# SimonRennotte/Data-Efficient-Reinforcement-Learning-with-Probabilistic-Model-Predictive-Control

Measured on AMD Instinct MI355X. Metric: MPC trajectory rollouts/sec, higher is better.
Workload: dtype f64

## Files before the change

### data-efficient-reinforcement-learning-with-probabilistic-model-predictive-control_amd/_lib.py

```python
import ctypes as C
import os

_HERE = os.path.dirname(os.path.abspath(__file__))
LIB_PATH = os.environ.get("GPMPC_LIB") or os.path.join(_HERE, "libgpmpc_hip.so")

GPMPC_OK = 0
GPMPC_ERR_ARG = -1
GPMPC_ERR_NOT_PD = -2
GPMPC_ERR_HIP = -3
GPMPC_ERR_LIMIT = -4


class GpmpcError(RuntimeError):
    def __init__(self, code, msg):
        super().__init__(f"gpmpc error {code}: {msg}")
        self.code = code


class NotPositiveDefiniteError(GpmpcError):
    """Cholesky failure of K + noise*I -- the reference lets torch.linalg.cholesky's error
    propagate uncaught (rl_gp_mpc/control_objects/models/gp_model.py:427)."""


_P = C.c_void_p
# ... 49 lines not shown
    "gpmpc_lbfgs_state_size": (C.c_longlong, [_I, _I, _I]),
    "gpmpc_lbfgs_init": (C.c_int, [_P, _P, _I, _I, _I, _I, _I, _P, _P, _P, _P]),
    "gpmpc_lbfgs_step": (C.c_int, [_P, _P, _P, _I, _I, _I, _I, _I, _D, _D, _I, _P, _P, _P, _P]),
    "gpmpc_lbfgs_search": (C.c_int, [_P, _P, _P, _I, _I, _I, _I, _D, _I, _I, _I, _I, _D, _D, _I, _P, _P, _P, _P, _P, _P]),
    "gpmpc_mll_batch": (C.c_int, [_P, _P, _P, _I, _I, _I, _P, _I, _P, _P, _I, _P, _P, _P, _P, _P]),
    "gpmpc_train_search": (C.c_int, [_P, _P, _P, _I, _I, _I, _I, _P, _P, _I, _I, _I, _I, _D, _D, _P, _P, _P, _P]),
    "gpmpc_ilqr_state_size": (C.c_longlong, [_I, _I, _I, _I, _I]),
    "gpmpc_ilqr_backward": (C.c_int, [_P, _P, _P, _I, _I, _I, _I, _D, _P, _P, _P, _P, _P, _P]),
    "gpmpc_ilqr_forward": (C.c_int, [_P, _P, _P, _P, _P, _P, _I, _I, _I, _I, _D, _P, _I, _P, _P, _P, _P]),
    "gpmpc_ilqr_init": (C.c_int, [_P, _P, _I, _I, _I, _I, _D, _P, _P]),
    "gpmpc_ilqr_step": (C.c_int, [_P, _P, _I, _I, _I, _I, _D, _I, _D, _D, _D, _D, _P, _P]),
    "gpmpc_ilqr_search": (C.c_int, [_P, _P, _P, _I, _I, _I, _I, _D, _I, _I, _D, _D, _D, _D, _P, _P, _P, _P]),
    "gpmpc_argmin_async": (C.c_int, [_P, _P, _I, C.c_longlong, _P, _I, _P, _P]),
    "gpmpc_argmin_export": (C.c_int, [_P, _P, _I, C.c_longlong, _P, _I, _P, _P, _P]),
    "gpmpc_argmin": (C.c_int, [_P, _P, _I, C.c_longlong, C.POINTER(_D), C.POINTER(C.c_longlong), _P]),
}


ABI_VERSION = 29


def load(path=LIB_PATH):
    if not os.path.exists(path):
        raise ImportError(
            f"{path} not found: the HIP extension is required (no CPU fallback). "
            "Build it with `python __graft_entry__.py` or `make -C <package>/csrc`.")
    lib = C.CDLL(path)
    for name, (res, args) in SIGNATURES.items():
        fn = getattr(lib, name)
        fn.restype = res
        fn.argtypes = args
    if lib.gpmpc_abi_version() != ABI_VERSION:
        raise ImportError(f"{path}: ABI version {lib.gpmpc_abi_version()} != expected {ABI_VERSION}; rebuild the HIP library")
    return lib
# ... 11 lines not shown
```

### data-efficient-reinforcement-learning-with-probabilistic-model-predictive-control_amd/csrc/abi.hip

```cpp
#include <climits>
#include <cmath>
#include <cstring>
#include <new>
#include <dlfcn.h>

#include "gpmpc_internal.h"
#include "lqr_gains_plan.h"
#include "lbfgs_state.h"
#include "ilqr_state.h"

namespace {
struct Roctx {
    int (*push)(const char*) = nullptr;
    int (*pop)() = nullptr;
    Roctx() {
        for (const char* lib : {"librocprofiler-sdk-roctx.so", "libroctx64.so"}) {
            void* hnd = dlopen(lib, RTLD_LAZY | RTLD_LOCAL);
            if (!hnd) continue;
            push = reinterpret_cast<int (*)(const char*)>(dlsym(hnd, "roctxRangePushA"));
            pop = reinterpret_cast<int (*)()>(dlsym(hnd, "roctxRangePop"));
            if (push && pop) return;
            push = nullptr; pop = nullptr;
        }
    }
// ... 105 lines not shown
}

template <class Run>
static int query_entry(gpmpc_t* g, const char* name, const char* count_name, int count, int D, int E, bool check_limits,
                       bool have_ptrs, Run run) {
    int rc = query_checks(g, name, count_name, count, D, E, check_limits);
    if (rc) return rc;
    if (count > 0 && !have_ptrs) return bad(g, "null argument");
    if (count == 0) return GPMPC_OK;
    GPMPC_HIP_CHECK(H_(g), hipSetDevice(g->h.device));
    return run(H_(g));
}

extern "C" {

int gpmpc_abi_version(void) { return 29; }

int gpmpc_create(gpmpc_t** out, int device_id) {
    if (!out) return GPMPC_ERR_ARG;
    *out = nullptr;
    int ndev = 0;
    if (hipGetDeviceCount(&ndev) != hipSuccess || device_id < 0 || device_id >= ndev) return GPMPC_ERR_HIP;
    if (hipSetDevice(device_id) != hipSuccess) return GPMPC_ERR_HIP;
    gpmpc_t* g = new (std::nothrow) gpmpc();
    if (!g) return GPMPC_ERR_HIP;
    g->h.device = device_id;
    hipDeviceProp_t prop;
    if (hipGetDeviceProperties(&prop, device_id) == hipSuccess) {
        g->h.num_cu = prop.multiProcessorCount;
        if (prop.maxSharedMemoryPerMultiProcessor >= 64 * 1024)
            g->h.lds_limit = (int)prop.maxSharedMemoryPerMultiProcessor;
// ... 1 lines not shown
    }
    *out = g;
    return GPMPC_OK;
}

int gpmpc_destroy(gpmpc_t* g) {
    if (!g) return GPMPC_ERR_ARG;
    Handle* h = H_(g);
    (void)hipSetDevice(h->device);
    Buf* all[] = {&h->Xt, &h->beta, &h->iK, &h->Tm, &h->ils2, &h->var, &h->logvar, &h->gram,
                  &h->linv, &h->zvec, &h->cost, &h->best, &h->xrange, &h->mono_w, &h->traj, &h->Xc, &h->Yc,
                  &h->hyp, &h->kv, &h->vv, &h->sc, &h->gradws, &h->mllws, &h->mllbws, &h->trainws, &h->cemws, &h->tilews, &h->sepw, &h->tgradws, &h->xch, &h->hio, &h->predws, &h->predbws, &h->covws, &h->momws, &h->mombws, &h->linws, &h->linbws, &h->fbws, &h->fbbws, &h->lqrws, &h->lbfgsws, &h->ilqrws, &h->Xf, &h->Yf, &h->fgws, &h->spws, &h->sprec, &h->selws, &h->spupd};
    for (Buf* b : all) free_buf(*b);
    if (h->hio_host) (void)hipHostFree(h->hio_host);
    if (h->hio_flag) (void)hipHostFree(h->hio_flag);
    if (h->xch_uc) (void)hipFree(h->xch_uc);
    if (h->info) (void)hipFree(h->info);
    if (h->fidx) (void)hipFree(h->fidx);
    if (h->mono_exp) (void)hipFree(h->mono_exp);
    if (h->septab) (void)hipFree(h->septab);
    if (h->side_stream) (void)hipStreamDestroy(h->side_stream);
    if (h->ev_params) (void)hipEventDestroy(h->ev_params);
    if (h->ev_points) (void)hipEventDestroy(h->ev_points);
    delete g;
    return GPMPC_OK;
}

const char* gpmpc_last_error(const gpmpc_t* g) { return g ? g->h.err.c_str() : "null handle"; }

int gpmpc_set_option(gpmpc_t* g, const char* name, long long value) {
// ... 220 lines not shown
    memcpy(a.mu0, mu0, h->D * sizeof(double));
    memcpy(a.S0, S0, (size_t)h->D * h->D * sizeof(double));
    return GPMPC_OK;
}

static int rollout_entry(gpmpc_t* g, bool linear, const double* actions, const double* gains, int gains_per_candidate,
                         const double* mu0, const double* S0, int B, int H, int A, int include_time, double time0, double* mu_out,
                         double* Sig_out, double* cm_out, double* cv_out, double* J_out, void* stream) {
    if (!g) return GPMPC_ERR_ARG;
    RolloutArgs a;
    int rc = fill_args(g, a, actions, mu0, S0, B, H, A, include_time, time0, cm_out || cv_out || J_out);
    if (rc) return rc;
    if (gains && A < 1) return bad(g, "feedback gains need A >= 1");
    GPMPC_HIP_CHECK(H_(g), hipSetDevice(g->h.device));
    a.mu_out = mu_out; a.Sig_out = Sig_out; a.cm_out = cm_out; a.cv_out = cv_out; a.J_out = J_out;
    if (!linear) return launch_rollout(H_(g), a, (hipStream_t)stream);
    return run_rollout_linear(H_(g), a, (hipStream_t)stream, gains, gains && gains_per_candidate != 0);
}

int gpmpc_rollout(gpmpc_t* g, const double* actions, const double* mu0, const double* S0, int B, int H, int A,
                  int include_time, double time0, double* mu_out, double* Sig_out, double* cm_out, double* cv_out,
                  double* J_out, void* stream) {
    Range roctx_range("gpmpc_rollout");
    return rollout_entry(g, false, actions, nullptr, 0, mu0, S0, B, H, A, include_time, time0, mu_out, Sig_out, cm_out, cv_out, J_out,
                         stream);
}

int gpmpc_rollout_linear(gpmpc_t* g, const double* actions, const double* mu0, const double* S0, int B, int H, int A,
                         int include_time, double time0, double* mu_out, double* Sig_out, double* cm_out, double* cv_out,
                         double* J_out, void* stream) {
// ... 120 lines not shown
    if (!actions_bar_out) return bad(g, "null argument");
    if (!gains && gains_bar_out) return bad(g, "gains_bar_out without gains");
    RolloutSeeds sd{mu_bar, Sig_bar, cm_bar, cv_bar, J_bar, mu0_bar_out, S0_bar_out, cm_bar || cv_bar || J_bar};
    RolloutArgs a;
    int rc = fill_args(g, a, actions, mu0, S0, B, H, A, include_time, time0, sd.cost);
    if (rc) return rc;
    if (A < 1) return bad(g, "gradient needs A >= 1");
    if (a.D > GPMPC_MAX_D || a.E > GPMPC_MAX_E) {
        g->h.err = "rollout_feedback_backward: D or E beyond the compiled limits";
        return GPMPC_ERR_LIMIT;
    }
    GPMPC_HIP_CHECK(H_(g), hipSetDevice(g->h.device));
    return run_rollout_feedback_backward(H_(g), a, sd, gains, gains && gains_per_candidate != 0, actions_bar_out, gains_bar_out,
                                         (hipStream_t)stream);
}

namespace {
constexpr int kUploadMax = 480;
struct UploadArgs { double v[kUploadMax]; };
__global__ __launch_bounds__(64) void upload_kernel(double* dst, int n, const UploadArgs a) {
    for (int i = threadIdx.x; i < n; i += 64) dst[i] = a.v[i];
}
}

int gpmpc_objective_grad_host(gpmpc_t* g, const double* actions_host, const double* mu0, const double* S0, int H, int A,
                              int include_time, double time0, const double** result_host, void* stream) {
    Range roctx_range("gpmpc_objective_grad_host");
    if (!g) return GPMPC_ERR_ARG;
    if (!actions_host || !result_host) return bad(g, "null argument");
    Handle* h = H_(g);
// ... 42 lines not shown
    a.Sig_out = q; q += (size_t)(H + 1) * D * D;
    a.cm_out = q; q += H + 1;
    a.cv_out = q;
    const unsigned long long seq = ++h->hio_seq;
    const bool sweep_exports = D <= 8;
    h->hx_out = h->hio_host_dev; h->hx_src = out_dev; h->hx_n = sweep_exports ? (int)n_out : 0;
    rc = launch_rollout_grad(h, a, grad, s);
    h->hx_n = 0;
    if (rc) return rc;
    if (!sweep_exports) {
        GPMPC_HIP_CHECK(h, hipStreamSynchronize(s));
        GPMPC_HIP_CHECK(h, hipMemcpy(h->hio_host, out_dev, n_out * sizeof(double), hipMemcpyDeviceToHost));
        *result_host = h->hio_host;
        return GPMPC_OK;
    }
    volatile unsigned long long* flag = h->hio_flag;
    for (unsigned spins = 1; *flag != seq; ++spins) {
        __builtin_ia32_pause();
        if ((spins & 0xfff) == 0) {
            const hipError_t qe = hipStreamQuery(s);
            if (qe == hipSuccess) {
                if (*flag == seq) break;
                h->err = "objective_grad_host: the launches ended without the sweep's completion word";
                return GPMPC_ERR_HIP;
            }
            if (qe != hipErrorNotReady) GPMPC_HIP_CHECK(h, qe);
        }
    }
    __atomic_thread_fence(__ATOMIC_ACQUIRE);
    *result_host = h->hio_host;
    return GPMPC_OK;
}

int gpmpc_cem_search(gpmpc_t* g, const double* mu0, const double* S0, int B, int H, int A, int include_time, double time0,
                     int iterations, int n_elite, unsigned long long seed, const double* first_candidate, int mapper,
                     const double* max_change, const double* action_prev, const double* noise_dev, double* best_out_dev,
                     void* stream) {
    Range roctx_range("gpmpc_cem_search");
    if (!g) return GPMPC_ERR_ARG;
    if (!best_out_dev) return bad(g, "null argument");
    Handle* h = H_(g);
    if (!h->ready) return bad(g, "search before prepare / set_factors");
    RolloutArgs a;
    int rc = fill_args(g, a, best_out_dev, mu0, S0, B, H, A, include_time, time0);
// ... 285 lines not shown
                        double* out_host, void* stream) {
    Range roctx_range("gpmpc_argmin_export");
    if (!g || !J || !out_dev || !out_host || B < 1 || first < 0 || HA < 0) return bad(g, "bad argument");
    Handle* h = H_(g);
    GPMPC_HIP_CHECK(h, hipSetDevice(h->device));
    hipPointerAttribute_t attr;
    void* dev_view = nullptr;
    if (hipPointerGetAttributes(&attr, out_host) != hipSuccess || attr.type != hipMemoryTypeHost ||
        hipHostGetDevicePointer(&dev_view, out_host, 0) != hipSuccess || !dev_view) {
        (void)hipGetLastError();
        return bad(g, "out_host must be pinned (page-locked, device-mapped) host memory");
    }
    return launch_argmin_to(h, J, B, first, actions, HA, out_dev, static_cast<double*>(dev_view), (hipStream_t)stream);
}

static int sparse_update_entry(gpmpc_t* g, const char* name, const double* X, const double* Y, int k, int D, int E, bool forget,
                               void* stream) {
    if (!g) return GPMPC_ERR_ARG;
    Handle* h = H_(g);
    const std::string pre = std::string(name) + ": ";
    if (!h->ready || !h->sp_have) return bad(g, (pre + "the handle holds no record of a gpmpc_prepare_sparse").c_str());
    if (!X || !Y) return bad(g, "null argument");
    if (k < 1) return bad(g, (pre + "need k >= 1 points").c_str());
    if (D != h->D || E != h->E) return bad(g, (pre + "D and E must be those of the cached sparse model").c_str());
    GPMPC_HIP_CHECK(h, hipSetDevice(h->device));
    return run_sparse_update(h, X, Y, k, forget, (hipStream_t)stream);
}

int gpmpc_sparse_append(gpmpc_t* g, const double* Xnew, const double* Ynew, int k, int D, int E, void* stream) {
    Range roctx_range("gpmpc_sparse_append");
// ... 10 lines not shown
```

### data-efficient-reinforcement-learning-with-probabilistic-model-predictive-control_amd/csrc/gpmpc_internal.h

```cpp
#pragma once
#include <hip/hip_runtime.h>
#include <cstddef>
#include <cstdio>
#include <string>
#include <unordered_set>

#include "../../include/gpmpc.h"

namespace gpmpc_hip {

constexpr int kMaxD = GPMPC_MAX_D;
constexpr int kMaxE = GPMPC_MAX_E;
constexpr int kWave = 64;

struct ClusterMap {
    int CS, D, P, P_off, wpp, wtri, koff;
    int CSd;
    unsigned char sepown[8];
    unsigned char meanown[4];
    unsigned char dmem[32];
    unsigned char didx[32];
    __host__ __device__ int diag_owner(int ord, int slot) const { return dmem[((ord * wtri + slot) * CSd) / (D * wtri)]; }
    __host__ __device__ int off_owner(int ord, int slot) const { return ((slot * koff) / wpp + ord * koff) % CS; }
    __host__ __device__ int sep_owner(int ord) const { return sepown[ord]; }
// ... 94 lines not shown
    int t_begin, t_end;
    int ntiles;
    const double* tile_part;
    const int* slow;
    double* grad_mom;
    int* grad_done;
    int grad_NSP, grad_NXP;
    int cluster;
    ClusterMap cmap;
    int cl_slots;
    int xch_n;
    unsigned xch_tag0;
    unsigned long long* xch;
    unsigned long long* xch_uc;
    int cl_dbg;
    int act_inline_n;
    double* act_store;
    double act_inline[kInlineActs];
    double mu0[kMaxD];
    double S0[kMaxD * kMaxD];
};

inline void rollout_objective_only(RolloutArgs& a, const double* actions, double* J) {
    a.actions = actions;
    a.J_out = J;
    a.mu_out = nullptr; a.Sig_out = nullptr; a.cm_out = nullptr; a.cv_out = nullptr;
}

struct Buf {
    double* p = nullptr;
// ... 52 lines not shown
    bool have_state = false;
    Buf Xf, Yf;
    Buf fgws;
    Buf spws;
    Buf selws;
    int* fidx = nullptr;
    size_t fidx_cap = 0;
    Buf hio;
    double* hio_host = nullptr;
    double* hio_host_dev = nullptr;
    size_t hio_host_cap = 0;
    unsigned long long* hio_flag = nullptr;
    unsigned long long* hio_flag_dev = nullptr;
    unsigned long long hio_seq = 0;
    double* hx_out = nullptr; const double* hx_src = nullptr; int hx_n = 0;
    Buf xch;
    unsigned long long* xch_uc = nullptr;
    size_t xch_uc_cap = 0;
    unsigned xch_epoch = 1;
    int opt_cluster = 0;
    int opt_cl_dbg = 0;
    int last_cluster = 1;
    int last_pair_groups = 1;
    Buf mono_w;
    int* mono_exp = nullptr;
    int mono_D = -1;
    int mono_cum[16] = {0};
    int sep_kmax = 0;
    int mono_CM = 0;
    int* info = nullptr;
// ... 155 lines not shown
    SyrkInvForm syrk;
};

struct ForgetRows {
    int k;
    int few[8];
    const int* many;
};

int ensure_rollout_tables(Handle* h, int N, int D);
int plan_rollout(const Handle& h, int N, int D, int A, int E, int H, int Bp, const RolloutRequest& req, RolloutPlan& p);
int launch_rollout(Handle* h, RolloutArgs& a, const RolloutPlan& p, hipStream_t s);
int launch_rollout(Handle* h, RolloutArgs& a, hipStream_t s);
int launch_argmin(Handle* h, const double* J, int B, long long first, hipStream_t s);
int launch_traj_cost(Handle* h, const RolloutArgs& a, double* cm, double* cv, double* J, hipStream_t s);
int ensure_sep_table(Handle* h, int D);
bool tile_path_fits(const Handle& h, int N, int D, int E);
int tile_workspace(Handle* h, RolloutArgs& a);
int launch_tile_state_init(Handle* h, const RolloutArgs& a, hipStream_t s);
int launch_pair_tiles(Handle* h, const RolloutArgs& a, int t, hipStream_t s);
bool tile_moments_supported(const Handle& h, int D, int E, int NSP);
int launch_tile_moments(Handle* h, const RolloutArgs& a, double* mom, int* done, int NSP, int NXP, hipStream_t s);
struct RolloutSeeds {
    const double* mu; const double* Sig; const double* cm; const double* cv; const double* J;
    double* mu0_bar; double* S0_bar;
    bool cost;
};
int plan_rollout_grad(Handle* h, int N, int D, int A, int E, int H, int B, int Bp, bool seeded, GradPlan& p);
int launch_rollout_grad(Handle* h, RolloutArgs& a, double* grad_out, hipStream_t s, const RolloutSeeds* seeds = nullptr);
int launch_rollout_grad_wide(Handle* h, RolloutArgs& a, double* grad_out, hipStream_t s,
// ... 95 lines not shown
```

### data-efficient-reinforcement-learning-with-probabilistic-model-predictive-control_amd/csrc/moments_linear.hip

```cpp
#include "moments_linear_kernels.h"

namespace gpmpc_hip {

namespace {

struct LinFinishArgs {
    const double* part;
    const double* ils2;
    const double* var;
    const double* Sig;
    double* M_out;
    double* S_out;
    double* V_out;
    int rows, E, D, nCB, NW;
    long long Mc;
};

__global__ __launch_bounds__(64) void moments_linear_finish_kernel(LinFinishArgs p) {
    __shared__ double s_sum[kMaxD][kMaxE + 2];
    __shared__ double s_V[kMaxE][kMaxD];
    __shared__ double s_T[kMaxE][kMaxD];
    const int m = blockIdx.x, tid = threadIdx.x;
    const int D = p.D, E = p.E, NW = p.NW;
    const bool with_S = p.S_out != nullptr;
// ... 115 lines not shown
        }
        double ucb = -cm + kappa * sqrt(cv);
        if (clip) ucb = fmin(ucb, 0.0);
        jsum -= ucb;
        if (cm_out) cm_out[(size_t)c * (H + 1) + t] = cm;
        if (cv_out) cv_out[(size_t)c * (H + 1) + t] = cv;
    }
    jsum = wave_xor_sum(jsum);
    if (lane == 0 && J_out) J_out[c] = jsum / (double)(H + 1);
}

}

int launch_traj_cost_feedback(Handle* h, const RolloutArgs& a, int rows, const double* mu, const double* Sig, const double* actions,
                              const double* gains, long long gain_stride, double* cm, double* cv, double* J, hipStream_t s) {
    const int D = a.D, A = a.A, H = a.H;
    auto launch = [&](auto kernel) {
        hipLaunchKernelGGL(kernel, dim3(rows), dim3(64), 0, s, mu, Sig, actions, gains, gain_stride, a.cost, D, A, H, a.kappa,
                           a.clip, a.use_constraints, cm, cv, J);
    };
    static_assert(kMaxD <= 16, "traj_cost_feedback_kernel: per-lane arrays");
    if (D <= 4) launch(traj_cost_feedback_kernel<4>);
    else if (D <= 8) launch(traj_cost_feedback_kernel<8>);
    else launch(traj_cost_feedback_kernel<16>);
    GPMPC_HIP_CHECK(h, hipGetLastError());
    return GPMPC_OK;
}

int run_moments_linear(Handle* h, const double* mu, const double* Sig, int P, double* M_out, double* S_out, double* V_out,
                       hipStream_t s) {
// ... 89 lines not shown
```

### data-efficient-reinforcement-learning-with-probabilistic-model-predictive-control_amd/csrc/rollout.hip

```cpp
#include "rollout_stream_kernel.h"

namespace gpmpc_hip {

int launch_rollout_dp2(Handle*, RolloutArgs&, int, bool, size_t, hipStream_t);
int launch_rollout_dp3(Handle*, RolloutArgs&, int, bool, size_t, hipStream_t);
int launch_rollout_dp4(Handle*, RolloutArgs&, int, bool, size_t, hipStream_t);
int launch_rollout_dp6(Handle*, RolloutArgs&, int, bool, size_t, hipStream_t);
int launch_rollout_dp8(Handle*, RolloutArgs&, int, bool, size_t, hipStream_t);
int launch_rollout_dp16(Handle*, RolloutArgs&, int, bool, size_t, hipStream_t);

__global__ __launch_bounds__(64) void traj_cost_kernel(const double* __restrict__ mu, const double* __restrict__ Sig,
                                                       const double* __restrict__ actions, const double* __restrict__ cost,
                                                       int D, int A, int H, double kappa, int clip, int use_constraints,
                                                       double* __restrict__ cm_out, double* __restrict__ cv_out,
                                                       double* __restrict__ J_out) {
    traj_cost_body(blockIdx.x, threadIdx.x, mu, Sig, actions, cost, D, A, H, kappa, clip, use_constraints, cm_out, cv_out, J_out);
}

__device__ __forceinline__ void keep_better(double& bv, long long& bi, double ov, long long oi) {
    if (oi >= 0 && (bi < 0 || ov < bv || (ov == bv && oi < bi))) { bv = ov; bi = oi; }
}

__global__ __launch_bounds__(1024) void argmin_kernel(const double* J, int B, long long first, double* out, int index_as_double,
                                                     const double* actions, int HA, double* out_host) {
// ... 33 lines not shown
        if (index_as_double) out[1] = (double)gi;
        else reinterpret_cast<long long*>(out)[1] = gi;
        if (out_host) { out_host[0] = bv; out_host[1] = (double)gi; }
    }
    if (actions) {
        const long long w = bi < 0 ? 0 : bi;
        for (int k = tid; k < HA; k += nt) {
            const double v = actions[w * HA + k];
            out[2 + k] = v;
            if (out_host) out_host[2 + k] = v;
        }
    }
    if (out_host) __threadfence_system();
}

__global__ __launch_bounds__(256) void xch_zero_kernel(unsigned long long* p, size_t n) {
    for (size_t i = (size_t)blockIdx.x * 256 + threadIdx.x; i < n; i += (size_t)gridDim.x * 256)
        __hip_atomic_store(p + i, 0ull, __ATOMIC_RELAXED, __HIP_MEMORY_SCOPE_AGENT);
}

struct InlineActs { double v[kInlineActs]; };
__global__ __launch_bounds__(64) void inline_acts_kernel(double* dst, int n, const InlineActs a) {
    for (int i = threadIdx.x; i < n; i += 64) dst[i] = a.v[i];
}

static int zero_exchange(Handle* h, unsigned long long* p, size_t words, hipStream_t s) {
    const unsigned blocks = (unsigned)((words + 255) / 256 < 256 ? (words + 255) / 256 : 256);
    hipLaunchKernelGGL(xch_zero_kernel, dim3(blocks ? blocks : 1), dim3(256), 0, s, p, words);
    GPMPC_HIP_CHECK(h, hipGetLastError());
    return GPMPC_OK;
}

int launch_traj_cost(Handle* h, const RolloutArgs& a, double* cm, double* cv, double* J, hipStream_t s) {
    hipLaunchKernelGGL(traj_cost_kernel, dim3(a.B), dim3(64), 0, s, a.mu_out, a.Sig_out, a.actions, a.cost, a.D, a.A, a.H, a.kappa,
                       a.clip, a.use_constraints, cm, cv, J);
    GPMPC_HIP_CHECK(h, hipGetLastError());
    return GPMPC_OK;
}

static inline int argmin_threads(int B) {
    const int w = (B + 63) / 64;
    return 64 * (w < 1 ? 1 : w > 16 ? 16 : w);
}

int launch_argmin_to(Handle* h, const double* J, int B, long long first, const double* actions, int HA, double* out_dev,
                     double* out_host, hipStream_t s) {
    hipLaunchKernelGGL(argmin_kernel, dim3(1), dim3(argmin_threads(B)), 0, s, J, B, first, out_dev, 1, actions, HA, out_host);
    GPMPC_HIP_CHECK(h, hipGetLastError());
    return GPMPC_OK;
}

// ... 280 lines not shown
        }
    };
    if (tiled) {
        rc = tile_workspace(h, a);
        if (!rc) rc = launch_tile_state_init(h, a, s);
        for (int t = 0; t < a.H && !rc; ++t) {
            rc = launch_pair_tiles(h, a, t, s);
            a.t_begin = t; a.t_end = t + 1;
            if (!rc) rc = launch_kernel();
        }
    } else {
        rc = launch_kernel();
    }
    if (rc) return rc;
    if ((a.cm_out || a.cv_out || a.J_out) && !p.costs_to_caller) {
        rc = launch_traj_cost(h, a, a.cm_out, a.cv_out, a.J_out, s);
        if (rc) return rc;
    }
    h->last_rollout_path = p.path;
    h->last_cluster = p.cluster;
    {
        const int Pk = tiled ? a.D * (a.D - 1) / 2 : a.D * (a.D + 1) / 2;
        h->last_pair_groups = (p.path == 1 || p.G < 1 || Pk < 1) ? 1 : (Pk + p.G - 1) / p.G;
    }
    return GPMPC_OK;
}

int launch_rollout(Handle* h, RolloutArgs& a, hipStream_t s) {
    int rc = ensure_rollout_tables(h, a.N, a.D);
    if (rc) return rc;
    RolloutPlan p;
// ... 7 lines not shown
```

### data-efficient-reinforcement-learning-with-probabilistic-model-predictive-control_amd/engine.py

```python
import ctypes as C

import numpy as np
import torch

from . import _lib as L


def _host(a, shape=None):
    a = np.ascontiguousarray(np.asarray(a, dtype=np.float64))
    if shape is not None and a.shape != tuple(shape):
        raise ValueError(f"expected shape {tuple(shape)}, got {a.shape}")
    return a


def _hp(a):
    return a.ctypes.data_as(C.c_void_p)


def _ptr(t):
    return t.data_ptr() if t is not None else None


def feedback_gains_layout(shape, B, H, A, D):
    shape = tuple(int(s) for s in shape)
# ... 349 lines not shown
        actions = self._dev(actions)
        B, H, A = actions.shape
        D = self.D
        mu0 = _host(mu0, (D,))
        S0 = _host(S0, (D, D))
        gain_args = ()
        if closed_loop:
            gains, per_candidate = self._gains(gains, B, H, A, D)
            gain_args = (_ptr(gains), int(per_candidate))
        out = self._trajectory_out(out, B, H, D, A, trajectories, stage_costs)
        self._check(getattr(self.lib, "gpmpc_" + name)(
            self._h, actions.data_ptr(), *gain_args, _hp(mu0), _hp(S0), B, H, A, int(bool(include_time)), float(time0),
            _ptr(out.get("mu")), _ptr(out.get("Sig")), _ptr(out.get("cost_mu")), _ptr(out.get("cost_var")), _ptr(out.get("J")),
            self._stream()))
        setattr(self, "_keep_" + name, (actions, gains))
        return out

    def rollout(self, actions, mu0, S0, include_time=False, time0=0.0, trajectories=True, stage_costs=True, out=None):
        return self._rollout("rollout", actions, mu0, S0, include_time, time0, trajectories, stage_costs, out)

    def rollout_linear(self, actions, mu0, S0, include_time=False, time0=0.0, trajectories=True, stage_costs=True, out=None):
        return self._rollout("rollout_linear", actions, mu0, S0, include_time, time0, trajectories, stage_costs, out)

    def rollout_linear_feedback(self, actions, gains, mu0, S0, include_time=False, time0=0.0, trajectories=True, stage_costs=True,
                                out=None):
        return self._rollout("rollout_linear_feedback", actions, mu0, S0, include_time, time0, trajectories, stage_costs, out,
                             closed_loop=True, gains=gains)

    def lqr_gains(self, actions, mu0, include_time=False, time0=0.0, reg=0.0, want_cost_to_go=False, want_flags=False):
        actions = self._dev(actions)
# ... 479 lines not shown
        if out is None:
            out = torch.empty(2 + ha, dtype=torch.float64, device=self.device)
        if host_out is None:
            self._check(self.lib.gpmpc_argmin_async(self._h, J.data_ptr(), J.numel(), int(first_global_index),
                                                    None if actions is None else actions.data_ptr(), ha,
                                                    out.data_ptr(), self._stream()))
            return out
        if (host_out.device.type != "cpu" or host_out.dtype != torch.float64 or not host_out.is_contiguous()
                or host_out.numel() != 2 + ha or not host_out.is_pinned()):
            raise ValueError("host_out must be a pinned contiguous float64 host tensor of 2 + H*A elements")
        self._check(self.lib.gpmpc_argmin_export(self._h, J.data_ptr(), J.numel(), int(first_global_index),
                                                 None if actions is None else actions.data_ptr(), ha,
                                                 out.data_ptr(), host_out.data_ptr(), self._stream()))
        return out

    def argmin(self, J, first_global_index=0):
        J = self._dev(J)
        bj = C.c_double()
        bi = C.c_longlong()
        self._check(self.lib.gpmpc_argmin(self._h, J.data_ptr(), J.numel(), int(first_global_index), C.byref(bj),
                                          C.byref(bi), self._stream()))
        return float(bj.value), int(bi.value)
```

### data-efficient-reinforcement-learning-with-probabilistic-model-predictive-control_amd/sharding.py

```python
import math

import numpy as np
import torch
import torch.distributed as dist

LOCAL = "local"
CEM_MAX_RECORDS = 4096
_CEM_FAILED = 2147483646.0


def _active(group):
    return group is not LOCAL and dist.is_available() and dist.is_initialized()


def broadcast_from_first(array, device, group=None):
    a = np.ascontiguousarray(array, dtype=np.float64)
    if not _active(group):
        return a.copy()
    t = torch.as_tensor(a).to(device)
    src = dist.get_global_rank(group, 0) if group is not None else 0
    dist.broadcast(t, src=src, group=group)
    return t.cpu().numpy().reshape(a.shape)


# ... 115 lines not shown
    return ent[0]


_SIDE_STREAMS = {}


def side_stream(device):
    idx = torch.device(device).index
    if idx not in _SIDE_STREAMS:
        _SIDE_STREAMS[idx] = torch.cuda.Stream(device=device)
    return _SIDE_STREAMS[idx]


class PendingBest:

    def __init__(self, host, event, world, H, A, record=None, exchange_group=None):
        self.host, self.event, self.world, self.H, self.A = host, event, world, H, A
        self.record = record
        self.exchange_group = exchange_group
        self._result = None
        self._flat = None
        self.host_seconds = None

    def result(self):
        if self._result is not None:
            return self._result
        import time
        t0 = time.perf_counter()
        if self.event is not None:
            self.event.synchronize()
        host = self.host
        if self.exchange_group is not None:
            mine = host.clone()
            flat = torch.empty(self.world * mine.numel(), dtype=torch.float64)
            dist.all_gather_into_tensor(flat, mine, group=self.exchange_group)
            host = flat
        self._result = _winner_of(host.view(self.world, -1), self.world, self.H, self.A)
        self._flat = None
        self.host_seconds = time.perf_counter() - t0
        return self._result


def select_best_async(engine, J, actions_local, lo, num_candidates, group=None, host_buffer=None, record=None,
                      exchange="rccl"):
    n, H, A = actions_local.shape
    multi = _active(group)
    if (not multi and n > 0 and actions_local.device.type == "cuda" and getattr(engine, "argmin_exports_host", False)):
        if host_buffer is None or host_buffer.numel() != 2 + H * A:
            host_buffer = torch.empty(2 + H * A, dtype=torch.float64, pin_memory=True)
        rec = engine.argmin_async(J, first_global_index=lo, actions=actions_local, out=record, host_out=host_buffer)
        ev = torch.cuda.Event()
        ev.record(torch.cuda.current_stream(rec.device))
        return PendingBest(host_buffer, ev, 1, H, A, rec)
    rec = _local_record(engine, J, actions_local, lo, out=record)
    if exchange == "host" and multi:
        world = dist.get_world_size(group)
        xg = host_group(group)
        if rec.device.type != "cuda":
            return PendingBest(rec.clone(), None, world, H, A, rec, exchange_group=xg)
        if host_buffer is None or host_buffer.numel() != rec.numel():
            host_buffer = torch.empty(rec.numel(), dtype=torch.float64, pin_memory=True)
        host_buffer.copy_(rec, non_blocking=True)
        ev = torch.cuda.Event()
        ev.record(torch.cuda.current_stream(rec.device))
# ... 180 lines not shown
```

### include/gpmpc.h

```cpp
#ifndef GPMPC_H
#define GPMPC_H
#ifdef __cplusplus
extern "C" {
#endif

typedef struct gpmpc gpmpc_t;

enum {
    GPMPC_OK = 0,
    GPMPC_ERR_ARG = -1,
    GPMPC_ERR_NOT_PD = -2,
    GPMPC_ERR_HIP = -3,
    GPMPC_ERR_LIMIT = -4
};
#define GPMPC_MAX_D 16
#define GPMPC_MAX_E 24

int gpmpc_abi_version(void);
const char* gpmpc_build_id(void);
int gpmpc_create(gpmpc_t** out, int device_id);
int gpmpc_destroy(gpmpc_t* h);
const char* gpmpc_last_error(const gpmpc_t* h);

int gpmpc_prepare(gpmpc_t* h, const double* X_dev, const double* Y_dev, const double* lengthscales_dev,
// ... 101 lines not shown
                                    const double* mu0_host, const double* S0_host, int B, int H, int A, int include_time,
                                    double time0, const double* mu_bar_dev, const double* Sig_bar_dev,
                                    const double* cost_mu_bar_dev, const double* cost_var_bar_dev, const double* J_bar_dev,
                                    double* actions_bar_out_dev, double* gains_bar_out_dev, double* mu0_bar_out_dev,
                                    double* S0_bar_out_dev, void* stream);

int gpmpc_objective_grad_host(gpmpc_t* h, const double* actions_host, const double* mu0_host, const double* S0_host,
                              int H, int A, int include_time, double time0, const double** result_host, void* stream);

int gpmpc_argmin(gpmpc_t* h, const double* J_dev, int B, long long first_global_index, double* best_J_host,
                 long long* best_idx_host, void* stream);
int gpmpc_argmin_async(gpmpc_t* h, const double* J_dev, int B, long long first_global_index, const double* actions_dev, int HA,
                       double* out_dev, void* stream);
int gpmpc_argmin_export(gpmpc_t* h, const double* J_dev, int B, long long first_global_index, const double* actions_dev, int HA,
                        double* out_dev, double* out_host, void* stream);

int gpmpc_cem_search(gpmpc_t* h, const double* mu0_host, const double* S0_host, int B, int H, int A, int include_time, double time0,
                     int iterations, int n_elite, unsigned long long seed, const double* first_candidate_host, int mapper,
                     const double* max_change_host, const double* action_prev_host, const double* noise_dev, double* best_out_dev,
                     void* stream);
int gpmpc_cem_local(gpmpc_t* h, const double* mu0_host, const double* S0_host, int B_total, int first, int B_local, int H, int A,
                    int include_time, double time0, int iteration, int n_elite, unsigned long long seed,
                    const double* first_candidate_host, int mapper, const double* max_change_host, const double* action_prev_host,
                    const double* noise_dev, const double* state_dev, double* elites_out_dev, void* stream);
int gpmpc_cem_merge(gpmpc_t* h, const double* elites_dev, int lists, int n_elite, int n, int iteration, double* state_dev,
                    void* stream);

long long gpmpc_lbfgs_state_size(int B, int n, int history);
int gpmpc_lbfgs_init(gpmpc_t* h, const double* x0_dev, int B, int H, int A, int history, int mapper, const double* max_change_host,
                     const double* action_prev_host, double* state_dev, void* stream);
// ... 37 lines not shown
```

Baseline: 694,600.

## Fuse best-candidate argmin into trajectory cost kernel via armed ring of host slots

```diff
diff --git a/data-efficient-reinforcement-learning-with-probabilistic-model-predictive-control_amd/_lib.py b/data-efficient-reinforcement-learning-with-probabilistic-model-predictive-control_amd/_lib.py
--- a/data-efficient-reinforcement-learning-with-probabilistic-model-predictive-control_amd/_lib.py
+++ b/data-efficient-reinforcement-learning-with-probabilistic-model-predictive-control_amd/_lib.py
@@ -87,10 +87,16 @@
     "gpmpc_argmin_async": (C.c_int, [_P, _P, _I, C.c_longlong, _P, _I, _P, _P]),
     "gpmpc_argmin_export": (C.c_int, [_P, _P, _I, C.c_longlong, _P, _I, _P, _P, _P]),
     "gpmpc_argmin": (C.c_int, [_P, _P, _I, C.c_longlong, C.POINTER(_D), C.POINTER(C.c_longlong), _P]),
+    "gpmpc_best_arm": (C.c_int, [_P, C.c_longlong, _I, _P]),
+    "gpmpc_best_disarm": (C.c_int, [_P]),
+    "gpmpc_best_armed": (C.c_int, [_P, C.POINTER(_I), C.POINTER(C.c_longlong), C.POINTER(C.c_ulonglong)]),
+    "gpmpc_best_claim": (C.c_int, [_P, _P, _I, C.c_longlong, _P, _I, _P, C.POINTER(C.c_ulonglong)]),
+    "gpmpc_best_wait": (C.c_int, [_P, C.c_ulonglong, _I, _P]),
+    "gpmpc_best_peek": (C.c_int, [_P, C.c_ulonglong, _I, _P, _P]),
 }
 
 
-ABI_VERSION = 29
+ABI_VERSION = 30
 
 
 def load(path=LIB_PATH):
diff --git a/data-efficient-reinforcement-learning-with-probabilistic-model-predictive-control_amd/csrc/abi.hip b/data-efficient-reinforcement-learning-with-probabilistic-model-predictive-control_amd/csrc/abi.hip
--- a/data-efficient-reinforcement-learning-with-probabilistic-model-predictive-control_amd/csrc/abi.hip
+++ b/data-efficient-reinforcement-learning-with-probabilistic-model-predictive-control_amd/csrc/abi.hip
@@ -3,6 +3,7 @@
 #include <cstring>
 #include <new>
 #include <dlfcn.h>
+#include <sched.h>
 
 #include "gpmpc_internal.h"
 #include "lqr_gains_plan.h"
@@ -143,7 +144,7 @@
 
 extern "C" {
 
-int gpmpc_abi_version(void) { return 29; }
+int gpmpc_abi_version(void) { return 30; }
 
 int gpmpc_create(gpmpc_t** out, int device_id) {
     if (!out) return GPMPC_ERR_ARG;
@@ -175,6 +176,9 @@
     for (Buf* b : all) free_buf(*b);
     if (h->hio_host) (void)hipHostFree(h->hio_host);
     if (h->hio_flag) (void)hipHostFree(h->hio_flag);
+    if (h->best_host) (void)hipHostFree(h->best_host);
+    if (h->best_dev) (void)hipFree(h->best_dev);
+    if (h->best_count) (void)hipFree(h->best_count);
     if (h->xch_uc) (void)hipFree(h->xch_uc);
     if (h->info) (void)hipFree(h->info);
     if (h->fidx) (void)hipFree(h->fidx);
@@ -425,6 +429,7 @@
     if (gains && A < 1) return bad(g, "feedback gains need A >= 1");
     GPMPC_HIP_CHECK(H_(g), hipSetDevice(g->h.device));
     a.mu_out = mu_out; a.Sig_out = Sig_out; a.cm_out = cm_out; a.cv_out = cv_out; a.J_out = J_out;
+    a.best_tail = linear ? 0 : 1;
     if (!linear) return launch_rollout(H_(g), a, (hipStream_t)stream);
     return run_rollout_linear(H_(g), a, (hipStream_t)stream, gains, gains && gains_per_candidate != 0);
 }
@@ -575,6 +580,30 @@
     return run_rollout_feedback_backward(H_(g), a, sd, gains, gains && gains_per_candidate != 0, actions_bar_out, gains_bar_out,
                                          (hipStream_t)stream);
 }
+
+}
+
+namespace gpmpc_hip {
+int wait_host_word(Handle* h, const volatile unsigned long long* word, unsigned long long value, hipStream_t s, const char* what) {
+    for (unsigned spins = 1; *word != value; ++spins) {
+        __builtin_ia32_pause();
+        if ((spins & 0xfff) == 0) {
+            const hipError_t qe = hipStreamQuery(s);
+            if (qe == hipSuccess) {
+                if (*word == value) break;
+                h->err = std::string(what) + ": the launches ended without the completion word";
+                return GPMPC_ERR_HIP;
+            }
+            if (qe != hipErrorNotReady) GPMPC_HIP_CHECK(h, qe);
+            if ((spins & 0xffff) == 0) sched_yield();
+        }
+    }
+    __atomic_thread_fence(__ATOMIC_ACQUIRE);
+    return GPMPC_OK;
+}
+}
+
+extern "C" {
 
 namespace {
 constexpr int kUploadMax = 480;
@@ -647,20 +676,8 @@
         *result_host = h->hio_host;
         return GPMPC_OK;
     }
-    volatile unsigned long long* flag = h->hio_flag;
-    for (unsigned spins = 1; *flag != seq; ++spins) {
-        __builtin_ia32_pause();
-        if ((spins & 0xfff) == 0) {
-            const hipError_t qe = hipStreamQuery(s);
-            if (qe == hipSuccess) {
-                if (*flag == seq) break;
-                h->err = "objective_grad_host: the launches ended without the sweep's completion word";
-                return GPMPC_ERR_HIP;
-            }
-            if (qe != hipErrorNotReady) GPMPC_HIP_CHECK(h, qe);
-        }
-    }
-    __atomic_thread_fence(__ATOMIC_ACQUIRE);
+    rc = wait_host_word(h, h->hio_flag, seq, s, "objective_grad_host");
+    if (rc) return rc;
     *result_host = h->hio_host;
     return GPMPC_OK;
 }
@@ -976,6 +993,71 @@
     return launch_argmin_to(h, J, B, first, actions, HA, out_dev, static_cast<double*>(dev_view), (hipStream_t)stream);
 }
 
+static_assert(kBestSlots == GPMPC_BEST_SLOTS, "include/gpmpc.h documents the ring's length");
+int gpmpc_best_arm(gpmpc_t* g, long long first, int HA, void* stream) {
+    if (!g || first < 0 || HA < 0) return bad(g, "bad argument");
+    Handle* h = H_(g);
+    GPMPC_HIP_CHECK(h, hipSetDevice(h->device));
+    int rc = ensure_best_rings(h, HA, (hipStream_t)stream);
+    if (rc) return rc;
+    best_arm(h->best_ring, first, stream);
+    return GPMPC_OK;
+}
+
+int gpmpc_best_disarm(gpmpc_t* g) {
+    if (!g) return GPMPC_ERR_ARG;
+    best_disarm(H_(g)->best_ring);
+    return GPMPC_OK;
+}
+
+int gpmpc_best_armed(gpmpc_t* g, int* armed, long long* first, unsigned long long* issued) {
+    if (!g) return GPMPC_ERR_ARG;
+    const BestRing& r = H_(g)->best_ring;
+    if (armed) *armed = r.armed ? 1 : 0;
+    if (first) *first = r.first;
+    if (issued) *issued = r.issued;
+    return GPMPC_OK;
+}
+
+int gpmpc_best_claim(gpmpc_t* g, const double* J, int B, long long first, const double* actions, int HA, void* stream,
+                     unsigned long long* ticket) {
+    if (!g || !ticket) return bad(g, "null argument");
+    BestCall c;
+    c.J = J; c.actions = actions; c.B = B; c.HA = HA; c.first = first; c.stream = stream;
+    *ticket = best_claim(H_(g)->best_ring, c);
+    return GPMPC_OK;
+}
+
+int gpmpc_best_wait(gpmpc_t* g, unsigned long long ticket, int HA, double* record_host) {
+    Range roctx_range("gpmpc_best_wait");
+    if (!g || !record_host) return bad(g, "null argument");
+    Handle* h = H_(g);
+    if (best_overwritten(h->best_ring, ticket) || HA != h->best_HA || !h->best_host)
+        return bad(g, "best_wait: the ticket's ring slot has been handed to a later launch (read a selection before "
+                      "GPMPC_BEST_SLOTS further armed rollouts are enqueued)");
+    const double* slot = h->best_host + (size_t)best_slot_of(ticket) * best_slot_doubles(HA);
+    int rc = wait_host_word(h, reinterpret_cast<const volatile unsigned long long*>(slot), ticket,
+                            (hipStream_t)h->best_ring.stream, "best_wait");
+    if (rc) return rc;
+    memcpy(record_host, slot + 1, (size_t)(2 + HA) * sizeof(double));
+    return GPMPC_OK;
+}
+
+int gpmpc_best_peek(gpmpc_t* g, unsigned long long ticket, int HA, double* slot_dev_copy, double* slot_host_copy) {
+    if (!g || !slot_dev_copy || !slot_host_copy) return bad(g, "null argument");
+    Handle* h = H_(g);
+    if (best_overwritten(h->best_ring, ticket) || HA != h->best_HA || !h->best_host)
+        return bad(g, "best_peek: the ticket's ring slot has been handed to a later launch");
+    GPMPC_HIP_CHECK(h, hipSetDevice(h->device));
+    GPMPC_HIP_CHECK(h, hipStreamSynchronize((hipStream_t)h->best_ring.stream));
+    const size_t off = (size_t)best_slot_of(ticket) * best_slot_doubles(HA);
+    if (*reinterpret_cast<const volatile unsigned long long*>(h->best_host + off) != ticket)
+        return bad(g, "best_peek: the slot's completion word is not the ticket");
+    GPMPC_HIP_CHECK(h, hipMemcpy(slot_dev_copy, h->best_dev + off, (size_t)(2 + HA) * sizeof(double), hipMemcpyDeviceToHost));
+    memcpy(slot_host_copy, h->best_host + off + 1, (size_t)(2 + HA) * sizeof(double));
+    return GPMPC_OK;
+}
+
 static int sparse_update_entry(gpmpc_t* g, const char* name, const double* X, const double* Y, int k, int D, int E, bool forget,
                                void* stream) {
     if (!g) return GPMPC_ERR_ARG;
diff --git a/data-efficient-reinforcement-learning-with-probabilistic-model-predictive-control_amd/csrc/best_ring.h b/data-efficient-reinforcement-learning-with-probabilistic-model-predictive-control_amd/csrc/best_ring.h
--- /dev/null
+++ b/data-efficient-reinforcement-learning-with-probabilistic-model-predictive-control_amd/csrc/best_ring.h
@@ -0,0 +1,93 @@
+#pragma once
+#include <cstddef>
+
+namespace gpmpc_hip {
+
+constexpr int kBestSlots = 8;
+
+struct BestCall {
+    const void* J = nullptr;
+    const void* actions = nullptr;
+    int B = 0, HA = 0;
+    long long first = 0;
+    const void* stream = nullptr;
+};
+
+inline bool same_call(const BestCall& a, const BestCall& b) {
+    return a.J == b.J && a.actions == b.actions && a.B == b.B && a.HA == b.HA && a.first == b.first && a.stream == b.stream;
+}
+
+struct BestLaunch {
+    unsigned long long base = 0;
+    unsigned long long last = 0;
+    unsigned long long ticket = 0;
+    int slot = 0;
+};
+
+struct BestRing {
+    bool armed = false;
+    long long first = 0;
+    const void* stream = nullptr;
+    unsigned long long base = 0;
+    unsigned long long issued = 0;
+    BestCall last;
+    bool last_valid = false;
+    bool last_claimed = false;
+    int unclaimed = 0;
+};
+
+inline int best_slot_of(unsigned long long ticket) { return (int)(ticket % kBestSlots); }
+
+inline size_t best_slot_doubles(int HA) { return ((size_t)3 + (size_t)(HA > 0 ? HA : 0) + 7) / 8 * 8; }
+
+inline void best_arm(BestRing& r, long long first, const void* stream) {
+    r.armed = true; r.first = first; r.stream = stream; r.unclaimed = 0;
+    r.last_valid = false;
+}
+
+inline void best_disarm(BestRing& r) { r.armed = false; r.last_valid = false; r.unclaimed = 0; }
+
+inline void best_forget_last(BestRing& r) { r.last_valid = false; }
+
+inline bool best_wants_fused(BestRing& r, const void* stream) {
+    if (!r.armed) return false;
+    if (stream != r.stream) { r.last_valid = false; return false; }
+    if (r.last_valid && !r.last_claimed) {
+        if (++r.unclaimed >= 2) { best_disarm(r); return false; }
+    }
+    return true;
+}
+
+inline BestLaunch best_next(const BestRing& r, int B) {
+    BestLaunch l;
+    l.base = r.base;
+    l.last = r.base + (unsigned long long)B - 1ULL;
+    l.ticket = r.issued + 1ULL;
+    l.slot = best_slot_of(l.ticket);
+    return l;
+}
+
+inline void best_launched(BestRing& r, const BestLaunch& l, const BestCall& c) {
+    r.base = l.last + 1ULL;
+    r.issued = l.ticket;
+    r.last = c;
+    r.last_valid = true;
+    r.last_claimed = false;
+}
+
+inline unsigned long long best_claim(BestRing& r, const BestCall& want) {
+    if (!r.armed || !r.last_valid || r.last_claimed || !same_call(r.last, want)) return 0ULL;
+    r.last_claimed = true;
+    r.unclaimed = 0;
+    return r.issued;
+}
+
+inline void best_retire_all(BestRing& r) { r.issued += (unsigned long long)kBestSlots; r.last_valid = false; }
+
+inline bool best_is_last(const BestRing& r, unsigned long long ticket) { return r.last_valid && ticket == r.issued; }
+
+inline bool best_overwritten(const BestRing& r, unsigned long long ticket) {
+    return ticket == 0ULL || ticket > r.issued || r.issued - ticket >= (unsigned long long)kBestSlots;
+}
+
+}
diff --git a/data-efficient-reinforcement-learning-with-probabilistic-model-predictive-control_amd/csrc/gpmpc_internal.h b/data-efficient-reinforcement-learning-with-probabilistic-model-predictive-control_amd/csrc/gpmpc_internal.h
--- a/data-efficient-reinforcement-learning-with-probabilistic-model-predictive-control_amd/csrc/gpmpc_internal.h
+++ b/data-efficient-reinforcement-learning-with-probabilistic-model-predictive-control_amd/csrc/gpmpc_internal.h
@@ -6,6 +6,7 @@
 #include <unordered_set>
 
 #include "../../include/gpmpc.h"
+#include "best_ring.h"
 
 namespace gpmpc_hip {
 
@@ -132,6 +133,7 @@
     unsigned long long* xch;
     unsigned long long* xch_uc;
     int cl_dbg;
+    int best_tail;
     int act_inline_n;
     double* act_store;
     double act_inline[kInlineActs];
@@ -214,6 +216,12 @@
     unsigned long long* hio_flag_dev = nullptr;
     unsigned long long hio_seq = 0;
     double* hx_out = nullptr; const double* hx_src = nullptr; int hx_n = 0;
+    BestRing best_ring;
+    unsigned long long* best_count = nullptr;
+    double* best_dev = nullptr;
+    double* best_host = nullptr;
+    double* best_host_dev = nullptr;
+    int best_HA = -1;
     Buf xch;
     unsigned long long* xch_uc = nullptr;
     size_t xch_uc_cap = 0;
@@ -399,6 +407,9 @@
 int launch_rollout(Handle* h, RolloutArgs& a, hipStream_t s);
 int launch_argmin(Handle* h, const double* J, int B, long long first, hipStream_t s);
 int launch_traj_cost(Handle* h, const RolloutArgs& a, double* cm, double* cv, double* J, hipStream_t s);
+int launch_traj_cost_best(Handle* h, const RolloutArgs& a, double* cm, double* cv, double* J, hipStream_t s);
+int ensure_best_rings(Handle* h, int HA, hipStream_t s);
+int wait_host_word(Handle* h, const volatile unsigned long long* word, unsigned long long value, hipStream_t s, const char* what);
 int ensure_sep_table(Handle* h, int D);
 bool tile_path_fits(const Handle& h, int N, int D, int E);
 int tile_workspace(Handle* h, RolloutArgs& a);
diff --git a/data-efficient-reinforcement-learning-with-probabilistic-model-predictive-control_amd/csrc/moments_linear.hip b/data-efficient-reinforcement-learning-with-probabilistic-model-predictive-control_amd/csrc/moments_linear.hip
--- a/data-efficient-reinforcement-learning-with-probabilistic-model-predictive-control_amd/csrc/moments_linear.hip
+++ b/data-efficient-reinforcement-learning-with-probabilistic-model-predictive-control_amd/csrc/moments_linear.hip
@@ -153,6 +153,7 @@
 
 int launch_traj_cost_feedback(Handle* h, const RolloutArgs& a, int rows, const double* mu, const double* Sig, const double* actions,
                               const double* gains, long long gain_stride, double* cm, double* cv, double* J, hipStream_t s) {
+    best_forget_last(h->best_ring);
     const int D = a.D, A = a.A, H = a.H;
     auto launch = [&](auto kernel) {
         hipLaunchKernelGGL(kernel, dim3(rows), dim3(64), 0, s, mu, Sig, actions, gains, gain_stride, a.cost, D, A, H, a.kappa,
diff --git a/data-efficient-reinforcement-learning-with-probabilistic-model-predictive-control_amd/csrc/rollout.hip b/data-efficient-reinforcement-learning-with-probabilistic-model-predictive-control_amd/csrc/rollout.hip
--- a/data-efficient-reinforcement-learning-with-probabilistic-model-predictive-control_amd/csrc/rollout.hip
+++ b/data-efficient-reinforcement-learning-with-probabilistic-model-predictive-control_amd/csrc/rollout.hip
@@ -1,3 +1,5 @@
+#include <cstring>
+
 #include "rollout_stream_kernel.h"
 
 namespace gpmpc_hip {
@@ -71,6 +73,59 @@
     if (out_host) __threadfence_system();
 }
 
+struct BestTail {
+    unsigned long long* count;
+    unsigned long long last;
+    unsigned long long ticket;
+    long long first;
+    double* rec_dev;
+    unsigned long long* word_host;
+};
+
+__global__ __launch_bounds__(64) void traj_cost_best_kernel(const double* __restrict__ mu, const double* __restrict__ Sig,
+                                                            const double* __restrict__ actions, const double* __restrict__ cost,
+                                                            int D, int A, int H, double kappa, int clip, int use_constraints,
+                                                            double* __restrict__ cm_out, double* __restrict__ cv_out,
+                                                            double* J_out, const BestTail bt) {
+    const int lane = threadIdx.x;
+    traj_cost_body(blockIdx.x, lane, mu, Sig, actions, cost, D, A, H, kappa, clip, use_constraints, cm_out, cv_out, J_out);
+    unsigned long long drawn = 0;
+    if (lane == 0)
+        drawn = __hip_atomic_fetch_add(bt.count, 1ULL, __ATOMIC_ACQ_REL, __HIP_MEMORY_SCOPE_AGENT);
+    drawn = __shfl(drawn, 0, 64);
+    if (drawn != bt.last) return;
+    __builtin_amdgcn_fence(__ATOMIC_ACQUIRE, "agent");
+    const int B = gridDim.x, HA = H * A;
+    const double j0 = __hip_atomic_load(J_out, __ATOMIC_RELAXED, __HIP_MEMORY_SCOPE_AGENT);
+    double bv = INFINITY;
+    long long bi = -1;
+    for (int i = lane; i < B; i += 64) {
+        const double v = __hip_atomic_load(J_out + i, __ATOMIC_RELAXED, __HIP_MEMORY_SCOPE_AGENT);
+        if (v < bv) { bv = v; bi = i; }
+    }
+    for (int off = 32; off >= 1; off >>= 1) {
+        const double ov = __shfl_xor(bv, off, 64);
+        const long long oi = __shfl_xor(bi, off, 64);
+        keep_better(bv, bi, ov, oi);
+    }
+    if (bt.first == 0 && j0 != j0) { bv = j0; bi = 0; }
+    if (bi < 0) bv = INFINITY;
+    double* rec_host = reinterpret_cast<double*>(bt.word_host) + 1;
+    if (lane == 0) {
+        const double gi = (double)((bi < 0) ? -1 : bi + bt.first);
+        bt.rec_dev[0] = bv; bt.rec_dev[1] = gi;
+        rec_host[0] = bv; rec_host[1] = gi;
+    }
+    const long long w = bi < 0 ? 0 : bi;
+    for (int k = lane; k < HA; k += 64) {
+        const double v = actions[w * HA + k];
+        bt.rec_dev[2 + k] = v;
+        rec_host[2 + k] = v;
+    }
+    __threadfence_system();
+    if (lane == 0) __hip_atomic_store(bt.word_host, bt.ticket, __ATOMIC_RELEASE, __HIP_MEMORY_SCOPE_SYSTEM);
+}
+
 __global__ __launch_bounds__(256) void xch_zero_kernel(unsigned long long* p, size_t n) {
     for (size_t i = (size_t)blockIdx.x * 256 + threadIdx.x; i < n; i += (size_t)gridDim.x * 256)
         __hip_atomic_store(p + i, 0ull, __ATOMIC_RELAXED, __HIP_MEMORY_SCOPE_AGENT);
@@ -89,9 +144,50 @@
 }
 
 int launch_traj_cost(Handle* h, const RolloutArgs& a, double* cm, double* cv, double* J, hipStream_t s) {
+    best_forget_last(h->best_ring);
     hipLaunchKernelGGL(traj_cost_kernel, dim3(a.B), dim3(64), 0, s, a.mu_out, a.Sig_out, a.actions, a.cost, a.D, a.A, a.H, a.kappa,
                        a.clip, a.use_constraints, cm, cv, J);
     GPMPC_HIP_CHECK(h, hipGetLastError());
+    return GPMPC_OK;
+}
+
+int ensure_best_rings(Handle* h, int HA, hipStream_t s) {
+    if (!h->best_count) {
+        GPMPC_HIP_CHECK(h, hipMalloc(reinterpret_cast<void**>(&h->best_count), sizeof(unsigned long long)));
+        GPMPC_HIP_CHECK(h, hipMemset(h->best_count, 0, sizeof(unsigned long long)));
+        h->best_ring.base = 0;
+    }
+    if (h->best_HA == HA && h->best_dev && h->best_host) return GPMPC_OK;
+    GPMPC_HIP_CHECK(h, hipStreamSynchronize(s));
+    best_retire_all(h->best_ring);
+    if (h->best_dev) GPMPC_HIP_CHECK(h, hipFree(h->best_dev));
+    if (h->best_host) GPMPC_HIP_CHECK(h, hipHostFree(h->best_host));
+    h->best_dev = nullptr; h->best_host = nullptr; h->best_host_dev = nullptr; h->best_HA = -1;
+    const size_t bytes = (size_t)kBestSlots * best_slot_doubles(HA) * sizeof(double);
+    GPMPC_HIP_CHECK(h, hipMalloc(reinterpret_cast<void**>(&h->best_dev), bytes));
+    GPMPC_HIP_CHECK(h, hipHostMalloc(reinterpret_cast<void**>(&h->best_host), bytes, hipHostMallocMapped | hipHostMallocCoherent));
+    GPMPC_HIP_CHECK(h, hipHostGetDevicePointer(reinterpret_cast<void**>(&h->best_host_dev), h->best_host, 0));
+    memset(h->best_host, 0, bytes);
+    h->best_HA = HA;
+    return GPMPC_OK;
+}
+
+int launch_traj_cost_best(Handle* h, const RolloutArgs& a, double* cm, double* cv, double* J, hipStream_t s) {
+    const int HA = a.H * a.A;
+    int rc = ensure_best_rings(h, HA, s);
+    if (rc) return rc;
+    const BestLaunch l = best_next(h->best_ring, a.B);
+    const size_t stride = best_slot_doubles(HA);
+    BestTail bt;
+    bt.count = h->best_count; bt.last = l.last; bt.ticket = l.ticket; bt.first = h->best_ring.first;
+    bt.rec_dev = h->best_dev + (size_t)l.slot * stride;
+    bt.word_host = reinterpret_cast<unsigned long long*>(h->best_host_dev + (size_t)l.slot * stride);
+    hipLaunchKernelGGL(traj_cost_best_kernel, dim3(a.B), dim3(64), 0, s, a.mu_out, a.Sig_out, a.actions, a.cost, a.D, a.A, a.H,
+                       a.kappa, a.clip, a.use_constraints, cm, cv, J, bt);
+    GPMPC_HIP_CHECK(h, hipGetLastError());
+    BestCall c;
+    c.J = J; c.actions = a.actions; c.B = a.B; c.HA = HA; c.first = h->best_ring.first; c.stream = s;
+    best_launched(h->best_ring, l, c);
     return GPMPC_OK;
 }
 
@@ -402,7 +498,11 @@
     }
     if (rc) return rc;
     if ((a.cm_out || a.cv_out || a.J_out) && !p.costs_to_caller) {
-        rc = launch_traj_cost(h, a, a.cm_out, a.cv_out, a.J_out, s);
+        if (a.best_tail && a.J_out && best_wants_fused(h->best_ring, s)) {
+            rc = launch_traj_cost_best(h, a, a.cm_out, a.cv_out, a.J_out, s);
+        } else {
+            rc = launch_traj_cost(h, a, a.cm_out, a.cv_out, a.J_out, s);
+        }
         if (rc) return rc;
     }
     h->last_rollout_path = p.path;
diff --git a/data-efficient-reinforcement-learning-with-probabilistic-model-predictive-control_amd/engine.py b/data-efficient-reinforcement-learning-with-probabilistic-model-predictive-control_amd/engine.py
--- a/data-efficient-reinforcement-learning-with-probabilistic-model-predictive-control_amd/engine.py
+++ b/data-efficient-reinforcement-learning-with-probabilistic-model-predictive-control_amd/engine.py
@@ -387,6 +387,8 @@
             _ptr(out.get("mu")), _ptr(out.get("Sig")), _ptr(out.get("cost_mu")), _ptr(out.get("cost_var")), _ptr(out.get("J")),
             self._stream()))
         setattr(self, "_keep_" + name, (actions, gains))
+        J = out.get("J")
+        self._best_call = (J, J._version, actions, actions._version) if name == "rollout" and J is not None else None
         return out
 
     def rollout(self, actions, mu0, S0, include_time=False, time0=0.0, trajectories=True, stage_costs=True, out=None):
@@ -896,6 +898,44 @@
                                                  out.data_ptr(), host_out.data_ptr(), self._stream()))
         return out
 
+    _best_call = None
+
+    def claim_best(self, J, actions, first_global_index=0):
+        call, self._best_call = self._best_call, None
+        ha = int(actions[0].numel())
+        ticket = C.c_ulonglong(0)
+        if (call is not None and J.dtype == torch.float64 and J.is_contiguous() and actions.is_contiguous()
+                and J.data_ptr() == call[0].data_ptr() and J._version == call[1] and J.numel() == actions.shape[0]
+                and actions.data_ptr() == call[2].data_ptr() and actions._version == call[3]
+                and actions.shape == call[2].shape):
+            self._check(self.lib.gpmpc_best_claim(self._h, J.data_ptr(), J.numel(), int(first_global_index), actions.data_ptr(), ha,
+                                                  self._stream(), C.byref(ticket)))
+        if ticket.value:
+            return int(ticket.value)
+        self._check(self.lib.gpmpc_best_arm(self._h, int(first_global_index), ha, self._stream()))
+        return 0
+
+    def best_wait(self, ticket, host_out):
+        if host_out.device.type != "cpu" or host_out.dtype != torch.float64 or not host_out.is_contiguous():
+            raise ValueError("host_out must be a contiguous float64 host tensor of 2 + H*A elements")
+        self._check(self.lib.gpmpc_best_wait(self._h, int(ticket), host_out.numel() - 2, host_out.data_ptr()))
+        return host_out
+
+    def best_peek(self, ticket, ha):
+        dev = torch.empty(2 + ha, dtype=torch.float64)
+        host = torch.empty(2 + ha, dtype=torch.float64)
+        self._check(self.lib.gpmpc_best_peek(self._h, int(ticket), int(ha), dev.data_ptr(), host.data_ptr()))
+        return dev, host
+
+    def best_armed(self):
+        armed, first, issued = C.c_int(0), C.c_longlong(0), C.c_ulonglong(0)
+        self._check(self.lib.gpmpc_best_armed(self._h, C.byref(armed), C.byref(first), C.byref(issued)))
+        return bool(armed.value), int(first.value), int(issued.value)
+
+    def best_disarm(self):
+        self._best_call = None
+        self._check(self.lib.gpmpc_best_disarm(self._h))
+
     def argmin(self, J, first_global_index=0):
         J = self._dev(J)
         bj = C.c_double()
diff --git a/data-efficient-reinforcement-learning-with-probabilistic-model-predictive-control_amd/sharding.py b/data-efficient-reinforcement-learning-with-probabilistic-model-predictive-control_amd/sharding.py
--- a/data-efficient-reinforcement-learning-with-probabilistic-model-predictive-control_amd/sharding.py
+++ b/data-efficient-reinforcement-learning-with-probabilistic-model-predictive-control_amd/sharding.py
@@ -153,10 +153,11 @@
 
 class PendingBest:
 
-    def __init__(self, host, event, world, H, A, record=None, exchange_group=None):
+    def __init__(self, host, event, world, H, A, record=None, exchange_group=None, claim=None):
         self.host, self.event, self.world, self.H, self.A = host, event, world, H, A
         self.record = record
         self.exchange_group = exchange_group
+        self.claim = claim
         self._result = None
         self._flat = None
         self.host_seconds = None
@@ -166,6 +167,8 @@
             return self._result
         import time
         t0 = time.perf_counter()
+        if self.claim is not None:
+            self.claim[0].best_wait(self.claim[1], self.host)
         if self.event is not None:
             self.event.synchronize()
         host = self.host
@@ -187,6 +190,10 @@
     if (not multi and n > 0 and actions_local.device.type == "cuda" and getattr(engine, "argmin_exports_host", False)):
         if host_buffer is None or host_buffer.numel() != 2 + H * A:
             host_buffer = torch.empty(2 + H * A, dtype=torch.float64, pin_memory=True)
+        claim = getattr(engine, "claim_best", None)
+        ticket = claim(J, actions_local, lo) if claim is not None else 0
+        if ticket:
+            return PendingBest(host_buffer, None, 1, H, A, record, claim=(engine, ticket))
         rec = engine.argmin_async(J, first_global_index=lo, actions=actions_local, out=record, host_out=host_buffer)
         ev = torch.cuda.Event()
         ev.record(torch.cuda.current_stream(rec.device))
diff --git a/include/gpmpc.h b/include/gpmpc.h
--- a/include/gpmpc.h
+++ b/include/gpmpc.h
@@ -139,6 +139,15 @@
                        double* out_dev, void* stream);
 int gpmpc_argmin_export(gpmpc_t* h, const double* J_dev, int B, long long first_global_index, const double* actions_dev, int HA,
                         double* out_dev, double* out_host, void* stream);
+
+#define GPMPC_BEST_SLOTS 8
+int gpmpc_best_arm(gpmpc_t* h, long long first_global_index, int HA, void* stream);
+int gpmpc_best_disarm(gpmpc_t* h);
+int gpmpc_best_armed(gpmpc_t* h, int* armed, long long* first_global_index, unsigned long long* last_ticket);
+int gpmpc_best_claim(gpmpc_t* h, const double* J_dev, int B, long long first_global_index, const double* actions_dev, int HA,
+                     void* stream, unsigned long long* ticket);
+int gpmpc_best_wait(gpmpc_t* h, unsigned long long ticket, int HA, double* record_host);
+int gpmpc_best_peek(gpmpc_t* h, unsigned long long ticket, int HA, double* slot_dev_copy_host, double* slot_host_copy_host);
 
 int gpmpc_cem_search(gpmpc_t* h, const double* mu0_host, const double* S0_host, int B, int H, int A, int include_time, double time0,
                      int iterations, int n_elite, unsigned long long seed, const double* first_candidate_host, int mapper,
```

After: 684,200. -1.5%, worse.
